# mschauer/ZigZagBoomerang.jl

Measured on AMD Instinct MI355X. Metric: reflection events/sec, d=16384 local ZigZag (spdmp), ensemble of independent chains, higher is better.
Workload: dtype f64

## Files before the change

include/pdmp_debug.h:

```cpp
#ifndef PDMP_DEBUG_H
#define PDMP_DEBUG_H

#include <stddef.h>

#include "pdmp_mi355.h"

#ifdef __cplusplus
extern "C" {
#endif

#define PDMP_DEBUG_KERNEL_AUTO 0
#define PDMP_DEBUG_KERNEL_SEQ 1
#define PDMP_DEBUG_KERNEL_SPEC4 2
#define PDMP_DEBUG_KERNEL_SPEC8 3
#define PDMP_DEBUG_KERNEL_EXACTP 4
pdmp_status pdmp_debug_set_kernel(pdmp_ensemble* ens, int kernel);
pdmp_status pdmp_debug_set_spec_g2(pdmp_ensemble* ens, int on);
pdmp_status pdmp_debug_set_phase_profile(pdmp_ensemble* ens, int on);
pdmp_status pdmp_debug_phase_profile(pdmp_ensemble* ens, double* out16, int* kind);
pdmp_status pdmp_debug_set_track_groups(pdmp_ensemble* ens, int which);
pdmp_status pdmp_debug_set_helper_wave(pdmp_ensemble* ens, int mode);
pdmp_status pdmp_debug_set_track_lines(pdmp_ensemble* ens, int mode);
pdmp_status pdmp_debug_buffer_addresses(pdmp_ensemble* ens, uint64_t* out8);
pdmp_status pdmp_debug_placement(pdmp_ensemble* ens, char* buf, size_t nbuf);
pdmp_status pdmp_debug_set_placement(pdmp_ensemble* ens, int tune, int place, const char* rec, const char* kp, const char* ev);
pdmp_status pdmp_debug_move_buffer(pdmp_ensemble* ens, int which);
pdmp_status pdmp_debug_set_helper_steering(pdmp_ensemble* ens, double gain, int target, double ahead);
pdmp_status pdmp_debug_set_launch_count_limit(pdmp_ensemble* ens, uint32_t n);
pdmp_status pdmp_debug_set_consumer_overlap(pdmp_ensemble* ens, int mode);
pdmp_status pdmp_debug_host_drain_probe(pdmp_ensemble* ens, int64_t bytes, double* gbps);
pdmp_status pdmp_debug_last_kernel(pdmp_ensemble* ens, char* out, int64_t cap);
pdmp_status pdmp_debug_set_logistic_rows(pdmp_ensemble* ens, int row_width);
pdmp_status pdmp_debug_set_proposal_dump(pdmp_ensemble* ens, int64_t n);

pdmp_status pdmp_debug_math_probe(int device, uint64_t seed, int64_t n, double* out);

#define PDMP_MATH_U01 0
#define PDMP_MATH_LOG 1
#define PDMP_MATH_EXP 2
#define PDMP_MATH_SINCOS 3
#define PDMP_MATH_SINCOS2PI 4
#define PDMP_MATH_RANDN 5
#define PDMP_MATH_RANDN2 6
#define PDMP_MATH_RANDINT 7
#define PDMP_MATH_DIV 8
#define PDMP_MATH_SQRT 9
#define PDMP_MATH_PT_DEV 16
#define PDMP_MATH_PT_DEV_L 17
#define PDMP_MATH_PT_BPS 18
#define PDMP_MATH_PT_BPS_L 19
#define PDMP_MATH_PT_D1 20
#define PDMP_MATH_PT_G 21
#define PDMP_MATH_PT_G_L 22
#define PDMP_MATH_PT_Q 23
// ... 40 lines not shown
```

zigzagboomerang.jl_amd/_lib.py:

```python
import ctypes as C
import os

import numpy as np

from . import build as _build

PDMP_OK = 0
ABI_VERSION = 3
ERR_NAMES = {0: "PDMP_OK", 1: "PDMP_ERR_INVALID", 2: "PDMP_ERR_NO_DEVICE", 3: "PDMP_ERR_HIP",
             4: "PDMP_ERR_UNSUPPORTED", 5: "PDMP_ERR_NOMEM"}

PDMP_ERR_INVALID, PDMP_ERR_NO_DEVICE, PDMP_ERR_HIP, PDMP_ERR_UNSUPPORTED, PDMP_ERR_NOMEM = 1, 2, 3, 4, 5
SAMPLER_ZIGZAG_LOCAL, SAMPLER_ZIGZAG_ALL, SAMPLER_BPS, SAMPLER_STICKY_ZIGZAG, SAMPLER_BARRIER_ZIGZAG = 0, 1, 2, 3, 4
BARRIER_RULES = {"sticky": 0, "reflect": 1, "reversible": 2}
BARRIER_FN_PT3_L, BARRIER_FN_HIT, BARRIER_FN_RATES = 0, 1, 2
CHAIN_OK, CHAIN_BOUND_VIOLATED, CHAIN_STALLED, CHAIN_TRACE_FULL, CHAIN_PAUSED = 0, 1, 2, 3, 4


def needs_rerun(status):
    st = np.asarray(status)
    return bool(np.any((st == CHAIN_TRACE_FULL) | (st == CHAIN_PAUSED)))
RUN_REFERENCE_TAIL, RUN_STOP_BEFORE = 0, 1

EVENT_DTYPE = np.dtype([("t", "<f8"), ("i", "<i8"), ("x", "<f8"), ("theta", "<f8")])
COUNTERS_DTYPE = np.dtype([("t_last", "<f8"), ("num", "<u8"), ("nacc", "<u8"), ("nrefresh", "<u8"),
                           ("ntrace", "<u8"), ("nevents", "<u8"), ("ndraw_main", "<u8"),
                           ("ndraw_global", "<u8"), ("status", "<u4"), ("reserved", "<u4")])
assert EVENT_DTYPE.itemsize == 32 and COUNTERS_DTYPE.itemsize == 72

EXPORTED_SYMBOLS = [
    "pdmp_last_error", "pdmp_abi_version", "pdmp_device_count", "pdmp_ensemble_create",
    "pdmp_ensemble_destroy", "pdmp_ensemble_set_flow_zigzag", "pdmp_ensemble_set_target_gaussian_csc",
    "pdmp_ensemble_set_state", "pdmp_ensemble_set_state_synthetic", "pdmp_ensemble_run", "pdmp_ensemble_run_partitioned", "pdmp_ensemble_sync",
    "pdmp_ensemble_last_run_ms", "pdmp_ensemble_counters", "pdmp_ensemble_totals", "pdmp_ensemble_trace_copy",
    "pdmp_ensemble_trace_reset", "pdmp_ensemble_final_state", "pdmp_ensemble_batch_means",
    "pdmp_ensemble_trace_dev", "pdmp_ensemble_counters_dev", 
    "pdmp_ensemble_set_flow_bps", "pdmp_ensemble_set_state_bps", "pdmp_ensemble_bps_trace_copy",
    "pdmp_ensemble_bps_final_state", "pdmp_ensemble_set_sticky", "pdmp_ensemble_set_adaptscale", "pdmp_ensemble_final_sigma", "pdmp_ensemble_set_flow_boomerang", "pdmp_ensemble_set_local_bound", "pdmp_ensemble_set_target_logistic", "pdmp_ensemble_set_flow_factboomerang",
    "pdmp_ensemble_set_mass_cholesky", "pdmp_ensemble_set_bps_options", "pdmp_ensemble_set_bps_moments", "pdmp_ensemble_bps_moments",
    "pdmp_ensemble_set_bps_sticky", "pdmp_ensemble_bps_trace_free_copy", "pdmp_ensemble_bps_final_sticky",
    "pdmp_ensemble_set_flow_bps_modern", "pdmp_ensemble_set_bps_record_limit", "pdmp_ensemble_set_target_bps_logistic",
    "pdmp_ensemble_set_barriers", "pdmp_ensemble_final_barrier", "pdmp_ensemble_set_target_diffusion_bridge",
    "pdmp_ensemble_ess_begin", "pdmp_ensemble_ess_batch", "pdmp_ensemble_ess_end", "pdmp_ensemble_set_gradient_tracking",
    "pdmp_ensemble_path_integrals", "pdmp_ensemble_set_path_integrals", "pdmp_ensemble_set_neighbourhood", "pdmp_ensemble_info",
    "pdmp_ensemble_consume_begin", "pdmp_ensemble_consume", "pdmp_ensemble_consume_async", "pdmp_ensemble_last_consume_ms", "pdmp_ensemble_consume_mean", "pdmp_ensemble_consume_inclusion", "pdmp_ensemble_consume_discretized", "pdmp_ensemble_consume_cummean", "pdmp_ensemble_consume_cummean_copy", "pdmp_ensemble_subtrace_copy", "pdmp_1d_run",
    "pdmp_ensemble_bps_consume_begin", "pdmp_ensemble_bps_consume", "pdmp_ensemble_bps_consume_mean", "pdmp_ensemble_bps_consume_inclusion",
    "pdmp_ensemble_bps_consume_discretized", "pdmp_ensemble_bps_consume_cummean", "pdmp_ensemble_bps_consume_cummean_copy",
    "pdmp_ensemble_consume_condition", "pdmp_ensemble_consume_conditioned", "pdmp_ensemble_bps_consume_condition", "pdmp_ensemble_bps_consume_conditioned",
    "pdmp_ensemble_consume_pairs", "pdmp_ensemble_consume_pair_integrals", "pdmp_ensemble_bps_consume_pairs", "pdmp_ensemble_bps_consume_pair_integrals",
    "pdmp_comm_unique_id", "pdmp_comm_init", "pdmp_comm_destroy", "pdmp_comm_info", "pdmp_comm_barrier", "pdmp_comm_allreduce",
    "pdmp_ensemble_gather_traces", "pdmp_ensemble_reduce_moments", "pdmp_comm_gathered_copy",
    "pdmp_ensemble_gather_bps_traces", "pdmp_comm_gathered_bps_copy", "pdmp_ensemble_bps_trace_dev",
]
DEBUG_SYMBOLS = ["pdmp_debug_set_kernel", "pdmp_debug_set_spec_g2", "pdmp_debug_set_phase_profile", "pdmp_debug_phase_profile",
                 "pdmp_debug_set_proposal_dump", "pdmp_debug_set_track_groups", "pdmp_debug_set_helper_wave", "pdmp_debug_set_track_lines", "pdmp_debug_buffer_addresses", "pdmp_debug_placement", "pdmp_debug_set_placement", "pdmp_debug_move_buffer", "pdmp_debug_set_helper_steering", "pdmp_debug_set_launch_count_limit", "pdmp_debug_host_drain_probe", "pdmp_debug_set_consumer_overlap", "pdmp_debug_last_kernel", "pdmp_debug_set_logistic_rows", "pdmp_debug_math_probe", "pdmp_debug_math_eval", "pdmp_debug_write_probe", "pdmp_debug_sector_probe",
                 "pdmp_debug_sticky_eval", "pdmp_debug_trace_append", "pdmp_debug_barrier_eval", "pdmp_debug_bps_trace_append"]
DEBUG_KERNELS = {"auto": 0, "seq": 1, "spec4": 2, "spec8": 3, "exactp": 4}


class PdmpConfig(C.Structure):
    _fields_ = [("struct_size", C.c_uint32), ("device", C.c_int32), ("sampler", C.c_int32), ("adapt", C.c_int32),
                ("factor", C.c_double), ("nchains", C.c_int64), ("d", C.c_int64), ("trace_capacity", C.c_int64)]


class PdmpError(RuntimeError):
    def __init__(self, code, msg):
        super().__init__(f"{ERR_NAMES.get(code, code)}: {msg}")
        self.code = code


_lib = None
_loaded_path = None


def loaded_path():
    return _loaded_path


def lib_path():
    return os.environ.get("PDMP_MI355_LIB") or _build.LIB_PATH


def load():
    global _lib, _loaded_path
    if _lib is not None:
        return _lib
    path = lib_path()
    if not os.path.exists(path):
# ... 86 lines not shown
    L.pdmp_ensemble_set_local_bound.argtypes = [vp, C.c_int]
    L.pdmp_ensemble_set_gradient_tracking.argtypes = [vp, C.c_int]
    L.pdmp_ensemble_final_sigma.argtypes = [vp, i64, i64, vp]
    L.pdmp_ensemble_set_flow_bps.argtypes = [vp, vp, vp, vp, vp, f64, f64]
    L.pdmp_ensemble_set_flow_boomerang.argtypes = [vp, vp, vp, vp, vp, vp, f64, f64]
    L.pdmp_ensemble_set_state_bps.argtypes = [vp, f64, vp, vp, f64, vp]
    L.pdmp_ensemble_ess_begin.argtypes = [vp, f64]
    L.pdmp_ensemble_ess_batch.argtypes = [vp, f64]
    L.pdmp_ensemble_ess_end.argtypes = [vp, vp, vp, vp, vp, C.POINTER(i64), C.POINTER(f64), C.POINTER(f64)]
    L.pdmp_ensemble_set_mass_cholesky.argtypes = [vp, vp, vp, vp]
    L.pdmp_ensemble_set_bps_options.argtypes = [vp, C.c_int, C.c_int]
    L.pdmp_ensemble_set_bps_moments.argtypes = [vp, C.c_int]
    L.pdmp_ensemble_bps_moments.argtypes = [vp, f64, i64, i64, vp, vp]
    L.pdmp_ensemble_set_bps_sticky.argtypes = [vp, vp, C.c_int]
    L.pdmp_ensemble_bps_trace_free_copy.argtypes = [vp, i64, i64, i64, vp]
    L.pdmp_ensemble_bps_final_sticky.argtypes = [vp, i64, i64, vp, vp]
    L.pdmp_ensemble_set_flow_bps_modern.argtypes = [vp, C.c_double, C.c_double, vp, C.c_int]
    L.pdmp_ensemble_set_target_bps_logistic.argtypes = [vp, i64, vp, vp, vp, vp, vp, vp, vp, vp, f64]
    L.pdmp_ensemble_set_bps_record_limit.argtypes = [vp, i64]
    L.pdmp_debug_sticky_eval.argtypes = [C.c_int, C.c_int, i64, vp, vp, vp, vp]
    L.pdmp_debug_barrier_eval.argtypes = [C.c_int, C.c_int, i64, vp, vp, vp, vp]
    L.pdmp_ensemble_set_barriers.argtypes = [vp, vp, vp, vp, vp, vp, vp, C.c_int]
    L.pdmp_ensemble_final_barrier.argtypes = [vp, i64, i64, vp, vp]
    L.pdmp_debug_trace_append.argtypes = [vp, i64, vp, i64]
    L.pdmp_ensemble_bps_trace_copy.argtypes = [vp, i64, i64, i64, vp, vp, vp]
    L.pdmp_ensemble_bps_final_state.argtypes = [vp, i64, i64, vp, vp, vp, vp]
    L.pdmp_debug_set_kernel.argtypes = [vp, C.c_int]
    L.pdmp_debug_set_spec_g2.argtypes = [vp, C.c_int]
    L.pdmp_debug_set_phase_profile.argtypes = [vp, C.c_int]
    L.pdmp_debug_phase_profile.argtypes = [vp, vp, C.POINTER(C.c_int)]
    L.pdmp_debug_set_proposal_dump.argtypes = [vp, i64]
    L.pdmp_debug_set_track_groups.argtypes = [vp, C.c_int]
    L.pdmp_debug_set_helper_wave.argtypes = [vp, C.c_int]
    L.pdmp_debug_set_track_lines.argtypes = [vp, C.c_int]
    L.pdmp_debug_buffer_addresses.argtypes = [vp, C.POINTER(C.c_uint64)]
    L.pdmp_debug_move_buffer.argtypes = [vp, C.c_int]
    L.pdmp_debug_placement.argtypes = [vp, C.c_char_p, C.c_size_t]
    L.pdmp_debug_set_placement.argtypes = [vp, C.c_int, C.c_int, C.c_char_p, C.c_char_p, C.c_char_p]
    L.pdmp_debug_set_launch_count_limit.argtypes = [vp, C.c_uint32]
    L.pdmp_debug_set_helper_steering.argtypes = [vp, C.c_double, C.c_int, C.c_double]
    L.pdmp_debug_last_kernel.argtypes = [vp, C.c_char_p, i64]
    L.pdmp_debug_set_logistic_rows.argtypes = [vp, C.c_int]
    for name in EXPORTED_SYMBOLS + DEBUG_SYMBOLS:
        fn = getattr(L, name)
        if name not in ("pdmp_last_error", "pdmp_abi_version", "pdmp_device_count", "pdmp_ensemble_destroy", "pdmp_comm_destroy"):
            fn.restype = C.c_int
    _lib = L
    _loaded_path = path
    return L


class Config1d(C.Structure):
    _fields_ = [("struct_size", C.c_uint32), ("device", C.c_int32), ("flow", C.c_int32), ("adapt", C.c_int32), ("factor", C.c_double),
                ("nchains", C.c_int64), ("trace_capacity", C.c_int64), ("mu", C.c_double), ("sigma2", C.c_double), ("noise", C.c_double),
                ("b_sigma", C.c_double), ("b_mu", C.c_double), ("b_lambda", C.c_double)]


EVENT1D_DTYPE = np.dtype([("t", "<f8"), ("x", "<f8"), ("theta", "<f8")])
STATE1D_DTYPE = np.dtype([("t", "<f8"), ("x", "<f8"), ("theta", "<f8"), ("c", "<f8"), ("a", "<f8"), ("b", "<f8"), ("t_next", "<f8"),
                          ("t_ref", "<f8"), ("ndraw", "<u8"), ("num", "<i8"), ("acc", "<i8"), ("started", "<i4"), ("status", "<i4")])


def check(code):
    if code != PDMP_OK:
        raise PdmpError(code, load().pdmp_last_error().decode("utf-8", "replace"))

# ... 40 lines not shown
```

zigzagboomerang.jl_amd/csrc/pdmp_capi.hip:

```cpp
#include <algorithm>
#include <cstdarg>
#include <cstdio>
#include <cstring>

#include "pdmp_ensemble.hpp"

namespace {
thread_local std::string g_err;
thread_local std::string g_deferred_err;
}

pdmp_status fail(pdmp_status st, const char* fmt, ...) {
    char buf[512];
    va_list ap;
    va_start(ap, fmt);
    vsnprintf(buf, sizeof buf, fmt, ap);
    va_end(ap);
    g_err = buf;
    return st;
}
pdmp_status fail_hip(const char* expr, hipError_t err) {
    const std::string dm = g_deferred_err;
    g_deferred_err.clear();
    return fail(PDMP_ERR_HIP, "%s failed: %s%s%s", expr, hipGetErrorString(err), dm.empty() ? "" : " -- ", dm.c_str());
// ... 261 lines not shown
        return fail(PDMP_ERR_UNSUPPORTED, "PDMP_DEBUG_KERNEL_EXACTP: spdmp on a plain lattice (16 <= n <= 128, d >= 2048) with the bounding matrix equal to the target's, no adaptation, and a trace or no trace");
#endif
    const bool sticky_spec = sticky && e->use_spec && e->blob_mmax <= 16 && !dump;
    *fam = sticky ? (sticky_spec ? FAM_STICKY_SPEC : FAM_STICKY_RUN) : spec_ok ? FAM_SPEC : FAM_ONE_EVENT;
    return PDMP_OK;
}

pdmp_status ensemble_run_impl(pdmp_ensemble* e, double T, int flags, void* stream) {
    if (!e) return fail(PDMP_ERR_INVALID, "null argument");
    if (!e->has_state) return fail(PDMP_ERR_INVALID, "set_state must be called before run");
    if (e->trace_appended) return fail(PDMP_ERR_INVALID, "pdmp_debug_trace_append was used on this ensemble: its records no longer match its trace (set_state first)");
    if (flags != PDMP_RUN_REFERENCE_TAIL && flags != PDMP_RUN_STOP_BEFORE) return fail(PDMP_ERR_INVALID, "bad flags");
    HIP_TRY(hipSetDevice(e->cfg.device));
    e->ran = true;
    hipStream_t s = stream ? (hipStream_t)stream : e->stream;
    const int64_t n = e->cfg.nchains;
    const bool bps = e->cfg.sampler == PDMP_SAMPLER_BPS;
    if (!bps) e->dbg_phase_valid = 0;
    if (!bps && general_path(e) && e->lg_nemax >= 1024 && !e->d_hot.p) PDMP_TRY(e->d_hot.alloc((size_t)n * (size_t)e->cfg.d * 4));
    const pdmp::BpsRunParams B = bps_run_params(e, T, flags);
    pdmp::ZzRunParams P = run_params(e, T, flags);
    const pdmp::ZzGeneralParams Q = general_params(e);
    const pdmp::ZzLogisticTables LT = logistic_tables(e);
    KernelFamily fam;
    PDMP_TRY(select_family(e, P, Q, LT, &fam));
    const FamilyInfo& F = FAMILY[fam];
    DevBuf<double> dbgbuf, phbuf;
    const int64_t dbg_cap = bps ? 0 : e->dbg_dump;
    if (dbg_cap > 0) {
        PDMP_TRY(dbgbuf.alloc((size_t)dbg_cap * 16));
        HIP_TRY(hipMemsetAsync(dbgbuf.p, 0, (size_t)dbg_cap * 16 * sizeof(double), s));
        P.dbg = dbgbuf.p;
        P.dbg_cap = dbg_cap;
    }
    HIP_TRY(hipEventRecord(e->ev0, s));
    const bool profiled = e->dbg_phase != 0 && F.phase_kind != 0;
    if (profiled) {
        PDMP_TRY(phbuf.alloc(16));
        HIP_TRY(hipMemsetAsync(phbuf.p, 0, 16 * sizeof(double), s));
        P.dbg = phbuf.p;
        P.dbg_cap = 0;
    }
    int rc = 0;
    switch (fam) {
    case FAM_BPS:
        if (e->bps.modern && e->bps.logit) {
            e->last_kernel = "bps_logit_run_kernel";
            rc = pdmp::launch_bps_logit_run(B, bps_modern_params(e), bps_logit_params(e), n, s);
        } else if (e->bps.modern) {
            e->last_kernel = "bps_modern_run_kernel";
            rc = pdmp::launch_bps_modern_run(B, bps_modern_params(e), n, s);
        } else if (e->bps.sticky) {
            e->last_kernel = "bps_sticky_run_kernel";
            rc = pdmp::launch_bps_sticky_run(B, bps_sticky_params(e), n, s);
        } else {
            e->last_kernel = "bps_run_kernel";
            rc = pdmp::launch_bps_run(B, n, e->bps.diag, s, bps_moments_params(e));
        }
        break;
    case FAM_GENERAL: e->last_kernel = "zz_general_run_kernel"; rc = pdmp::launch_zz_general_run(P, Q, n, s); break;
    case FAM_LOGISTIC_LDS: e->last_kernel = "zz_logistic_lds_kernel"; rc = pdmp::launch_zz_logistic_lds(P, Q, LT, e->keep_integrals, n, s); break;
    case FAM_TRACKL: e->last_kernel = "zz_local_trackl_kernel"; e->canon_stale = true; rc = pdmp::launch_zz_local_trackl(P, n, s); break;
    case FAM_TRACKP: rc = pdmp::launch_zz_local_trackp(P, n, s, &e->last_kernel); break;
    case FAM_TRACK_GROUPS: e->last_kernel = "zz_local_track_kernel"; rc = pdmp::launch_zz_local_track(P, n, s); break;
    case FAM_STICKY_SPEC: e->last_kernel = "zz_sticky_spec_kernel"; rc = pdmp::launch_zz_sticky_spec(P, n, s); break;
    case FAM_STICKY_RUN: e->last_kernel = "zz_sticky_run_kernel"; rc = pdmp::launch_zz_sticky_run(P, n, s); break;
// ... 354 lines not shown
```

zigzagboomerang.jl_amd/csrc/pdmp_capi_debug.hip:

```cpp
#include <algorithm>
#include <chrono>
#include <cstdio>
#include <cstring>

#include "pdmp_ensemble.hpp"

template <class Launch>
static pdmp_status time_launches(const char* name, int iters, double* ms_out, Launch launch) {
    hipEvent_t e0, e1;
    HIP_TRY(hipEventCreate(&e0));
    HIP_TRY(hipEventCreate(&e1));
    (void)launch();
    HIP_TRY(hipEventRecord(e0, nullptr));
    for (int k = 0; k < iters; ++k) LAUNCH_TRY_CODE(name, launch());
    HIP_TRY(hipEventRecord(e1, nullptr));
    HIP_TRY(hipEventSynchronize(e1));
    float ms = 0.f;
    HIP_TRY(hipEventElapsedTime(&ms, e0, e1));
    *ms_out = (double)ms / iters;
    (void)hipEventDestroy(e0);
    (void)hipEventDestroy(e1);
    return PDMP_OK;
}

// ... 170 lines not shown
    if (!e || !e->has_state) return fail(PDMP_ERR_INVALID, "move buffer: an ensemble with a state");
    if ((which >= 6) != (e->cfg.sampler == PDMP_SAMPLER_BPS)) return fail(PDMP_ERR_INVALID, "move buffer: 6-10 are the Bouncy Particle's arrays, 0-5 the ZigZag's");
    HIP_TRY(device_sync(e));
    auto move_buf = [](auto& b) -> hipError_t {
        if (!b.p || b.n == 0) return hipSuccess;
        void* np = nullptr;
        const size_t bytes = b.n * sizeof(*b.p);
        hipError_t r = hipMalloc(&np, bytes);
        if (r != hipSuccess) return r;
        r = hipMemcpy(np, b.p, bytes, hipMemcpyDeviceToDevice);
        if (r != hipSuccess) return r;
        b.p = static_cast<decltype(b.p)>(np);
        return hipSuccess;
    };
    switch (which) {
        case 0: HIP_TRY(move_buf(e->d_rec)); break;
        case 1: HIP_TRY(move_buf(e->d_kp)); break;
        case 2: HIP_TRY(move_buf(e->d_ev)); break;
        case 3: HIP_TRY(move_buf(e->d_hdr)); break;
        case 4: HIP_TRY(move_buf(e->d_cc)); break;
        case 5: HIP_TRY(move_buf(e->d_keys)); break;
        case 6: HIP_TRY(move_buf(e->b_ev_x)); break;
        case 7: HIP_TRY(move_buf(e->b_ev_th)); break;
        case 8: HIP_TRY(move_buf(e->b_x)); break;
        case 9: HIP_TRY(move_buf(e->b_th)); break;
        case 10: HIP_TRY(move_buf(e->b_ev_t)); break;
        default: return fail(PDMP_ERR_INVALID, "move buffer: 0 records, 1 pairs, 2 trace, 3 headers, 4 constants, 5 keys; BPS: 6 / 7 event x / theta, 8 / 9 x / theta, 10 event t");
    }
    return PDMP_OK;
}
pdmp_status pdmp_debug_set_helper_wave(pdmp_ensemble* e, int mode) {
    if (!e || mode < -1 || mode > 1) return fail(PDMP_ERR_INVALID, "helper wave: -1 (by occupancy), 0 (never), 1 (always)");
    e->dbg_helper_wave = mode;
    return PDMP_OK;
}
pdmp_status pdmp_debug_set_consumer_overlap(pdmp_ensemble* e, int mode) {
    if (!e || mode < -1 || mode > 1) return fail(PDMP_ERR_INVALID, "consumer overlap: -1 (by width), 0 (between slices), 1 (beside the next slice)");
    e->dbg_cons_overlap = mode;
    return PDMP_OK;
}
pdmp_status pdmp_debug_set_launch_count_limit(pdmp_ensemble* e, uint32_t n) {
    if (!e) return fail(PDMP_ERR_INVALID, "null argument");
    e->dbg_count_limit = n;
    return PDMP_OK;
}
pdmp_status pdmp_debug_set_helper_steering(pdmp_ensemble* e, double gain, int target, double ahead) {
    if (!e || !(gain > 0.0 && gain <= 4096.0) || target < 1 || target > 64 || !(ahead >= 0.0))
        return fail(PDMP_ERR_INVALID, "helper steering: 0 < gain <= 4096 (<= 1 for the two-wave form), 1 <= target <= 64, ahead >= 0");
    e->dbg_hw_steer[0] = gain;
    e->dbg_hw_steer[1] = (double)target;
    e->dbg_hw_steer[2] = ahead;
    return PDMP_OK;
}
pdmp_status pdmp_debug_set_logistic_rows(pdmp_ensemble* e, int w) {
    if (!e || (w != -1 && w != 0 && w != 16 && w != 32)) return fail(PDMP_ERR_INVALID, "row width: -1 (default), 0 (one chain per wavefront), 16 or 32");
#ifndef PDMP_EXTRA_KERNELS
    if (w > 0) return fail(PDMP_ERR_UNSUPPORTED, "zz_logistic_rows_kernel is not part of this library: it lives in the parity build (build.py --variant parity, -DPDMP_EXTRA_KERNELS)");
#endif
    e->dbg_lg_rows = w;
    return PDMP_OK;
}
pdmp_status pdmp_debug_set_proposal_dump(pdmp_ensemble* e, int64_t n) {
    if (!e || n < 0) return fail(PDMP_ERR_INVALID, "bad argument");
    e->dbg_dump = n;
    return PDMP_OK;
}
// ... 111 lines not shown
```

zigzagboomerang.jl_amd/csrc/pdmp_engine.hpp:

```cpp
#pragma once
#include <cstdint>
#include <string>
#include <vector>

#include "../../include/pdmp_mi355.h"
#ifdef PDMP_EXTRA_KERNELS
#include "../../include/pdmp_debug.h"
#endif

namespace pdmp {

struct alignas(64) ZzRec {
    double x;
    double th;
    double t;
    double I;
    double t_old;
    double a, b;
    uint64_t acc;
};
static_assert(sizeof(ZzRec) == 64, "record must be one 64-byte sector");

struct alignas(128) TrRec {
    double x, th, tx, I;
// ... 41 lines not shown
    h.c.t_last = t0;
    h.c.num = 0;
    h.c.nacc = 0;
    h.c.nrefresh = 0;
    h.c.ntrace = ntrace;
    h.c.nevents = nevents;
    h.c.ndraw_main = ndraw_main;
    h.c.ndraw_global = 0;
    h.c.status = PDMP_CHAIN_OK;
    h.c.reserved = 0;
    h.seed = seed;
    h.t0 = t0;
    h.t_event = t0;
    h.tl_scale = 0.0;
    for (int k = 0; k < 3; ++k) h.pad[k] = 0;
    return h;
}

constexpr uint32_t PDMP_PRIO_TURN = 256u;
struct PrioTurn {
    uint32_t slot, it;
    __device__ __forceinline__ PrioTurn() : slot((uint32_t)__builtin_amdgcn_s_getreg(4 | (0 << 6) | (3 << 11)) & 3u), it(0) {}
    __device__ __forceinline__ void step() {
        if ((it & (PDMP_PRIO_TURN - 1u)) == 0u) {
            const uint32_t pr = ((it / PDMP_PRIO_TURN) + slot) & 3u;
            switch (pr) {
                case 0: __builtin_amdgcn_s_setprio(0); break;
                case 1: __builtin_amdgcn_s_setprio(1); break;
                case 2: __builtin_amdgcn_s_setprio(2); break;
                default: __builtin_amdgcn_s_setprio(3); break;
            }
        }
        it += 1;
    }
};
#endif

struct CoordConst {
    double c, c100;
    uint32_t cp, k;
    double gam[5];
};
static_assert(sizeof(CoordConst) == 64, "half a line");

struct BarrierEntry {
    double lo, hi;
    double klo, khi;
    uint32_t rules;
    uint32_t pad;
};
static_assert(sizeof(BarrierEntry) == 40, "barrier table entry");
constexpr uint64_t BARRIER_ACT_HIT = 0, BARRIER_ACT_REFLECT = 1, BARRIER_ACT_UNFREEZE = 2;

struct ZzTables {
    const uint32_t* __restrict__ colptr;
    const uint32_t* __restrict__ rowval;
    const double* __restrict__ bval;
    const double* __restrict__ tval;
    const double* __restrict__ gmu_b;
    const double* __restrict__ gmu_t;
    const uint32_t* __restrict__ sptr;
    const uint32_t* __restrict__ sidx;
    const uint32_t* __restrict__ qptr;
    const uint8_t* __restrict__ pos;
    const uint8_t* __restrict__ selfpos;
    const double* __restrict__ c_shared;
// ... 10 lines not shown
    ZzTables tb;
    ZzRec* rec;
    double* keys;
    DevChain* hdr;
    pdmp_event* ev;
    double* c_chain;
    double* dbg;
    int64_t dbg_cap;
    const uint64_t* __restrict__ blob;
    const uint32_t* __restrict__ tix;
    uint32_t blob_w, blob_w_pad, blob_sw, blob_pw, blob_kmax;
    uint32_t common_tix;
    int64_t d;
    int64_t dk;
    int64_t trace_cap;
    uint32_t nblk;
    uint32_t nblk_pad;
    double T;
    double factor;
    double lambda_ref;
    int32_t flags;
    int32_t adapt;
    int32_t has_refresh;
    int32_t move_all;
    int32_t force_spec4;
    int32_t track_two_sums;
    int32_t track_mean;
    uint32_t count_limit;
    uint32_t typ_extra;
    double hw_gain, hw_ahead;
    uint32_t hw_target;
    int32_t n_cu;
    int32_t helper_wave;
    void* tl_lines;
    void* tl_cold;
    int32_t lattice_n;
    uint32_t lattice_magic;
    const uint64_t* __restrict__ g8_line;
    const double* __restrict__ g8_member;
    const double* __restrict__ g8_gamt;
    int32_t g8_gw;
    const double* __restrict__ kappa;
    double* thf;
    int32_t reversible, strong_upperbounds;
    const BarrierEntry* __restrict__ barriers;
};

struct ZzInitParams {
    ZzTables tb;
    ZzRec* rec;
    double* keys;
    DevChain* hdr;
    double* c_chain;
    const double* x0;
    const double* th0;
    const uint64_t* seeds;
    uint64_t seed0;
    int64_t d;
    int64_t dk;
    int64_t nchains;
    double t0;
    double lambda_ref;
    int32_t has_refresh;
    int32_t sticky;
    double* thf;
    int32_t flow_kind;
// ... 340 lines not shown
```

zigzagboomerang.jl_amd/csrc/pdmp_ensemble.hpp:

```cpp
#pragma once
#include <hip/hip_runtime.h>

#include <cstdint>
#include <string>
#include <vector>

#include "../../include/pdmp_debug.h"
#include "pdmp_engine.hpp"

#pragma GCC visibility push(hidden)

pdmp_status fail(pdmp_status st, const char* fmt, ...);
pdmp_status fail_hip(const char* expr, hipError_t err);
pdmp_status fail_launch(const char* launcher, int rc, bool hip_rc);

#define HIP_TRY(expr)                                    \
    do {                                                 \
        hipError_t e_ = (expr);                          \
        if (e_ != hipSuccess) return fail_hip(#expr, e_); \
    } while (0)
#define LAUNCH_TRY_AS(name, rc, hip_rc)                            \
    do {                                                           \
        const int rc_ = (rc);                                      \
        if (rc_ != 0) return fail_launch(name, rc_, hip_rc);       \
// ... 176 lines not shown
    DevBuf<unsigned char> d_pr_cur, d_pr_meta;
    bool pr_on = false;
    int64_t pr_np = 0;
    bool trace_appended = false;
    DevBuf<pdmp_event> d_ev2;
    DevBuf<uint64_t> d_snap[2];
    hipStream_t stream2 = nullptr;
    hipEvent_t ev_run_done = nullptr, ev_cons_done[2] = {nullptr, nullptr}, ev_c0 = nullptr, ev_c1 = nullptr;
    bool cons_pending[2] = {false, false}, cons_timed = false;
    int async_k = 0;
    pdmp_event* deferred_buf = nullptr;
    int deferred_k = -1;

    DevBuf<double> d_jprev, d_sum, d_jstart, d_essacc;
    double ess_T0 = 0.0, ess_Tlast = 0.0;
    int64_t ess_batches = -1;

    pdmp::PlaceConfig place_cfg;
    int place_tune = 1;
    std::string tune_log;

    int dbg_kernel = 0;
    int dbg_lg_rows = -1;
    int dbg_spec_g2 = 0;
    int dbg_phase = 0;
    double dbg_phase_out[16] = {0};
    int dbg_phase_valid = 0;
    int64_t dbg_dump = 0;
    int dbg_track_groups = 0;
    double dbg_hw_steer[3] = {0, 0, 0};
    uint32_t dbg_count_limit = 0;
    int dbg_cons_overlap = -1;
    int dbg_helper_wave = -1;
    int dbg_track_lines = -1;

    BpsOptions bps;
    DevBuf<int64_t> b_colptr, b_rowval, bt_colptr, bt_rowval;
    DevBuf<double> b_nzval, b_mu, b_mu_flow, b_x, b_th, b_scal, b_ev_t, b_ev_x, b_ev_th, bt_nzval, bt_mu;
    DevBuf<int32_t> m_Lcp, m_Lrv, m_Ucp, m_Urv;
    DevBuf<double> m_Lnz, m_Unz;
    DevBuf<double> b_j1, b_j2;
    DevBuf<double> b_jT, b_jT2;
    DevBuf<double> b_kappa, b_thf, b_tfrez;
    DevBuf<uint64_t> b_fmask, b_ev_f;
    DevBuf<double> b_udiag, b_sudiag, b_mstate;
    DevBuf<int64_t> bl_Acp, bl_Arv, bl_Atcp, bl_Atrv;
    DevBuf<double> bl_Anz, bl_Atnz, bl_y, bl_m, bl_eta;
    int64_t bl_n = 0;
    double bl_gamma0 = 0.0;
    DevBuf<double> bc_cur, bc_grid, bc_cm;
    DevBuf<unsigned char> bc_meta;
    bool bc_on = false, bc_cummean = false;
    double bc_dt = 0.0;
    int64_t bc_K = 0;
    DevBuf<double> bcn_pn, bcn_tau, bcn_t, bcn_x;
    DevBuf<unsigned long long> bcn_nh;
    bool bcn_on = false, bc_started = false;
    int64_t bcn_max_hits = 0;

    DevBuf<int32_t> bpr_pi, bpr_pj;
    DevBuf<double> bpr_c, bpr_S, bpr_J, bpr_T;
    bool bpr_on = false;
    int64_t bpr_np = 0;

    pdmp::ZzTables tables() const {
        pdmp::ZzTables tb{};
// ... 64 lines not shown
```

zigzagboomerang.jl_amd/csrc/pdmp_trackp.hip:

```cpp
#include <hip/hip_runtime.h>

#include <cstdint>

#include "../../include/pdmp_detmath.h"
#include "pdmp_device.hpp"
#include "pdmp_engine.hpp"

namespace pdmp {

namespace {

__device__ __forceinline__ uint32_t w_grp8_min_u32(uint32_t v) {
    uint32_t o = (uint32_t)__builtin_amdgcn_mov_dpp((int)v, 0xB1, 0xf, 0xf, true);
    v = (o < v) ? o : v;
    o = (uint32_t)__builtin_amdgcn_mov_dpp((int)v, 0x4E, 0xf, 0xf, true);
    v = (o < v) ? o : v;
    o = (uint32_t)__builtin_amdgcn_mov_dpp((int)v, 0x141, 0xf, 0xf, true);
    return (o < v) ? o : v;
}
__device__ __forceinline__ uint32_t p_enc(double key, double tb, uint32_t pos) {
    double dlt = key - tb;
    dlt = (dlt > 0.0) ? dlt : 0.0;
    const uint32_t b = __float_as_uint((float)dlt);
    return (((b >= 8u) ? b - 8u : 0u) & ~7u) | pos;
// ... 11 lines not shown
    return reinterpret_cast<const uint32_t*>(smem)[b] & 7u;
}

}

template <bool HW, bool BIG = false>
struct WL {
    static_assert(!(HW && BIG), "the two-wave form keeps 2048 block bounds");
    static constexpr uint32_t NBLK = BIG ? 8192 : 2048;
    static constexpr uint32_t XO = (NBLK - 2048) * 4;
    static constexpr uint32_t LB = 0;
    static constexpr uint32_t EX = XO + 8192;
    static constexpr uint32_t URING = XO + 8704;
    static constexpr uint32_t SLB = XO + (HW ? 9792 : 9728);
    static constexpr uint32_t TB = XO + (HW ? 9920 : 9856);
    static constexpr uint32_t ACL = XO + (HW ? 10048 : 9984);
    static constexpr uint32_t NB = XO + (HW ? 10144 : 10016);
    static constexpr uint32_t CTL = 10272;
    static constexpr uint32_t HPF = 10336;
    static constexpr uint32_t RING = 10464;
    static constexpr int CMAX = HW ? 64 : 56;
    static constexpr uint32_t WIN = HW ? 256u : 128u;
    static constexpr uint32_t BYTES = HW ? RING + 512 * 16 : NB + 128;
};
constexpr uint32_t W_NR = 512;
constexpr uint32_t W_BYTES_1W = WL<false>::BYTES, W_BYTES_BIG = WL<false, true>::BYTES;
constexpr uint32_t W_BYTES_HW = WL<true>::BYTES;
constexpr int W_AMAX = 8;
#ifndef W_GROW
#define W_GROW 1.02
#define W_SHRINK 0.98
#define W_SLACK 5u
#endif
#define W_TARGET_HW 48u
#define W_GAIN_HW 0.3
#define W_TARGET_1W 44u
#define W_TARGET_1W_MAX_PER_CU 12
#define W_NHYP 8
#define W_NHYP_1W 4
#define W_PF_AHEAD 1.0
static_assert(WL<false>::BYTES <= 10240, "16 chains per CU: 160 KB / 16");
static_assert(WL<false>::URING + WL<false>::WIN * 8 <= WL<false>::SLB && WL<false, true>::URING + WL<false, true>::WIN * 8 <= WL<false, true>::SLB &&
                  WL<false>::ACL + W_AMAX * 2 <= WL<false>::NB,
              "the one-wave forms' ring of draws ends where the event blocks begin");
static_assert(WL<false, true>::BYTES <= 40960, "d <= 65536: 4 chains per CU (one per SIMD), 160 KB / 4");
static_assert(W_BYTES_HW == WL<true>::RING + W_NR * 16 && W_BYTES_HW <= 20480, "8 chains per CU: 160 KB / 8");
struct WCtl {
    uint32_t filled;
    uint32_t consumed;
    uint32_t exitf;
    uint32_t pad;
    double pf_tau, pf_dt, pf_tb;
};
typedef volatile __attribute__((address_space(3))) WCtl* WCtlPtr;
__device__ __forceinline__ WCtlPtr w_ctl(unsigned char* smem, uint32_t offset) {
    return (WCtlPtr)(__attribute__((address_space(3))) unsigned char*)(smem + offset);
}

namespace {
__device__ __forceinline__ bool nb_has(const uint4 nb, uint32_t v2) {
    const uint32_t x0 = nb.x ^ v2, x1 = nb.y ^ v2, x2 = nb.z ^ v2, x3 = nb.w ^ v2;
    const uint32_t z = ((x0 - 0x00010001u) & ~x0) | ((x1 - 0x00010001u) & ~x1) | ((x2 - 0x00010001u) & ~x2) | ((x3 - 0x00010001u) & ~x3);
    return (z & 0x80008000u) != 0u;
}
__device__ __forceinline__ uint32_t nb_count(const uint4 nb) {
    const uint64_t hi = ((uint64_t)nb.w << 32) | nb.z, lo = ((uint64_t)nb.y << 32) | nb.x;
// ... 107 lines not shown
    if (status == PDMP_CHAIN_BOUND_VIOLATED || status == PDMP_CHAIN_STALLED) return;
    const uint64_t seed = hdr->seed;
    const uint64_t nm0 = hdr->c.ndraw_main, ntrace0 = hdr->c.ntrace;
    if (HW) {
        if (threadIdx.x == 0) {
            ctl->filled = 0u;
            ctl->consumed = 0u;
            ctl->exitf = 0u;
            ctl->pf_tau = -PDMP_INF;
            ctl->pf_dt = 0.0;
            ctl->pf_tb = 0.0;
        }
        __syncthreads();
        if (threadIdx.x >= 64) {
            trackp_helper<LAT>(P, smem, lane, chain, seed, nm0);
            return;
        }
    }
    uint32_t dnm = 0, dnum = 0, dnacc = 0, vnacc = 0;
    double unext = 0.0;
    uint32_t ufilled = 0, uflushed = 0;
    bool uhave = false;
    double t_last = hdr->c.t_last;
    double t_event = hdr->t_event;
    status = PDMP_CHAIN_OK;
    const double T = P.T;
    const bool stop_before = (P.flags & PDMP_RUN_STOP_BEFORE) != 0;
    const uint32_t trace_room = (P.trace_cap > 0)
                                    ? (uint32_t)(((uint64_t)P.trace_cap > ntrace0) ? ((uint64_t)P.trace_cap - ntrace0) : 0)
                                    : 0xffffffffu;

    double seldt = 1e-3;
    double tb;
    {
        double mloc = t_last;
        for (uint32_t b = lane; b < nblk; b += 64) {
            const double2* p = kp + (size_t)b * 8;
#pragma unroll
            for (int q = 0; q < 8; ++q) mloc = min_f64(mloc, p[q].x);
        }
        tb = wave_min_f64(mloc);
    }
    for (uint32_t b = lane; b < W_NBLK; b += 64) {
        uint32_t e = P_INFBITS;
        if (b < nblk) {
            const double2* p = kp + (size_t)b * 8;
            double mk = p[0].x;
            uint32_t mi = 0;
#pragma unroll
            for (int q = 1; q < 8; ++q) {
                const double v = p[q].x;
                if (v < mk) {
                    mk = v;
                    mi = q;
                }
            }
            e = (mk < PDMP_INF) ? p_enc(mk, tb, mi) : P_INFBITS;
        }
        lbf[b] = e;
    }
    PDMP_LDS_ORDER();

    uint64_t ph[10] = {0, 0, 0, 0, 0, 0, 0, 0, 0, 0};
    uint64_t ph_t0 = PROF ? (uint64_t)__builtin_readcyclecounter() : 0;
    uint64_t ph_rounds = 0, ph_guess = 0;
    uint64_t ph_iters = 0, ph_raw = 0, ph_zone = 0, ph_eval = 0;
#ifdef PDMP_PHASE_MARKS
#define WMARK(k) asm volatile("; WPHASE " #k)
#else
#define WMARK(k)
#endif
#define WPHASE(k)                                                         \
    do {                                                                  \
        WMARK(k);                                                         \
        if (PROF) {                                                       \
            const uint64_t now_ = (uint64_t)__builtin_readcyclecounter(); \
            ph[k] += now_ - ph_t0;                                        \
            ph_t0 = now_;                                                 \
        }                                                                 \
    } while (0)

    PrioTurn prio;
    bool need_rebase = false;
    uint32_t idle = 0;
    bool running = stop_before || (t_event < T);
    while (running) {
        prio.step();
        if (dnacc >= trace_room) {
            status = PDMP_CHAIN_TRACE_FULL;
            break;
        }
        if (dnm >= P.count_limit) {
            status = PDMP_CHAIN_PAUSED;
            break;
        }
        if (HW) {
            if (lane == 0) ctl->consumed = dnm;
            while (ctl->filled < dnm + W_WIN) __builtin_amdgcn_s_sleep(1);
            PDMP_LDS_ORDER();
        } else {
            const uint32_t ulim = dnm + W_WIN;
            while (ufilled < ulim) {
                const uint32_t n = ufilled + (uint32_t)lane;
                if (!uhave) {
                    unext = pdmp_u01(seed, PDMP_STREAM_MAIN, nm0 + (uint64_t)n);
                    uhave = true;
                }
                const uint32_t uend = (ufilled + 64u < ulim) ? ufilled + 64u : ulim;
                if (n >= uflushed && n < uend) uring[n & (W_WIN - 1u)] = unext;
                uflushed = uend;
                if (uend != ufilled + 64u) break;
                ufilled += 64u;
                uhave = false;
            }
            PDMP_LDS_ORDER();
        }
        WPHASE(7);
        auto draw = [&](uint32_t n) -> double {
            if (HW) return ring[n & (W_NR - 1u)].x;
            return uring[n & (W_WIN - 1u)];
// ... 692 lines not shown
            const uint32_t costL = (uint32_t)__builtin_amdgcn_readlane((int)cost, (int)(Rc - 1u));
            const uint32_t offL = (uint32_t)__builtin_amdgcn_readlane((int)off, (int)(Rc - 1u));
            dnum += Rc;
            idle = 0;
            dnacc += (uint32_t)__popcll(acc_c);
            dnm += offL + costL;
            t_last = readlane_f64(tp, (int)(Rc - 1u));
            if (acc_c) t_event = readlane_f64(tp, 63 - __builtin_clzll(acc_c));
        }
        if (vsel >= 0) {
            const double tpv = readlane_f64(tp, vsel);
            const uint32_t iv = (uint32_t)__builtin_amdgcn_readlane((int)i, vsel);
            if (lane == 0) kp[iv].y = tpv;
            dnum += 1;
            vnacc = 1;
            dnm += 1;
            t_last = tpv;
            status = PDMP_CHAIN_BOUND_VIOLATED;
        }
        if (status != PDMP_CHAIN_OK) break;
        PDMP_LDS_ORDER();
    }

    if (PROF && P.dbg && chain == 0 && lane == 0) {
        for (int q = 0; q < 10; ++q) P.dbg[q] = (double)ph[q];
        P.dbg[10] = (double)ph_iters;
        P.dbg[11] = (double)ph_raw;
        P.dbg[12] = (double)ph_zone;
        P.dbg[13] = (double)ph_eval;
        P.dbg[14] = (double)ph_rounds;
        P.dbg[15] = (double)ph_guess;
    }
#undef WPHASE
    if (HW && lane == 0) ctl->exitf = 1u;
    if (lane == 0) {
        hdr->c.t_last = t_last;
        hdr->t_event = t_event;
        hdr->c.num += dnum;
        hdr->c.nacc += dnacc + vnacc;
        hdr->c.ntrace = ntrace0 + dnacc;
        hdr->c.nevents += dnacc;
        hdr->c.ndraw_main = nm0 + dnm;
        hdr->c.status = status;
    }
}

template <bool PROF, bool LAT>
__global__ __launch_bounds__(64) __attribute__((amdgpu_waves_per_eu(4, 4))) void zz_local_trackp_kernel(ZzRunParams P) {
    trackp_body<PROF, LAT, false, false>(P);
}
template <bool PROF>
__global__ __launch_bounds__(64) __attribute__((amdgpu_waves_per_eu(1, 2))) void zz_local_trackp_big_kernel(ZzRunParams P) {
    trackp_body<PROF, true, false, true>(P);
}
template <bool PROF, bool LAT>
__global__ __launch_bounds__(128) __attribute__((amdgpu_waves_per_eu(4, 4))) void zz_local_trackp2_kernel(ZzRunParams P) {
    trackp_body<PROF, LAT, true, false>(P);
}

bool zz_trackp_supported(const ZzRunParams& p) {
    const bool lattice = p.lattice_n >= 16 && p.lattice_n <= 256 && p.d <= (int64_t)WL<false, true>::NBLK * 8;
    const bool graph = p.lattice_n == 0 && p.tb.nb16 != nullptr && p.tb.gam8 != nullptr && p.d <= (int64_t)WL<false>::NBLK * 8;
    return (lattice || graph) && p.tb.gmu_t == nullptr && !p.track_two_sums && !p.has_refresh && p.d >= 2048;
}

bool zz_trackp_big(int64_t d) { return d > (int64_t)WL<false>::NBLK * 8; }
// ... 114 lines not shown
```

zigzagboomerang.jl_amd/engine.py:

```python
import ctypes as C
import os

import numpy as np

from . import _lib
from .flows import BouncyParticle, DiffusionBridgeTarget, FactBoomerang, GaussianTarget, LogisticRegressionTarget, LogisticTarget, ZigZag


def _i64(a):
    return np.ascontiguousarray(a, dtype=np.int64)


def _f64(a):
    return np.ascontiguousarray(a, dtype=np.float64)


def _ptr(a):
    return None if a is None else a.ctypes.data


class Ensemble:

    def __init__(self, nchains, d, *, sampler=_lib.SAMPLER_ZIGZAG_LOCAL, adapt=False, factor=1.8, device=0,
                 trace_capacity=0):
        self._L = _lib.load()
        self.nchains, self.d = int(nchains), int(d)
        self.trace_capacity = int(trace_capacity)
        self.adapt = bool(adapt)
        self.device = int(device)
        self._bps_mom = 0
        cfg = _lib.PdmpConfig(C.sizeof(_lib.PdmpConfig), int(device), int(sampler), int(bool(adapt)), float(factor),
                              self.nchains, self.d, self.trace_capacity)
        h = C.c_void_p()
        _lib.check(self._L.pdmp_ensemble_create(C.byref(cfg), C.byref(h)))
        self._h = h
        k = os.environ.get("PDMP_KERNEL")
        if k:
            self.debug_set_kernel(k)
        if os.environ.get("PDMP_TRACK_GROUPS"):
            _lib.check(self._L.pdmp_debug_set_track_groups(self._h, int(os.environ["PDMP_TRACK_GROUPS"])))
        if os.environ.get("PDMP_HELPER_WAVE"):
            self.debug_set_helper_wave(int(os.environ["PDMP_HELPER_WAVE"]))
        if os.environ.get("PDMP_TRACK_LINES"):
            self.debug_set_track_lines(int(os.environ["PDMP_TRACK_LINES"]))
        if any(os.environ.get(v) for v in ("PDMP_PLACE_TUNE", "PDMP_PLACE", "PDMP_PLACE_rec", "PDMP_PLACE_kp", "PDMP_PLACE_ev")):
            pat = [os.environ.get("PDMP_PLACE_" + a, "").encode() or None for a in ("rec", "kp", "ev")]
            self.debug_set_placement(int(os.environ.get("PDMP_PLACE_TUNE", "-1")), int(os.environ.get("PDMP_PLACE", "1" if any(pat) else "0")), *pat)
        if os.environ.get("PDMP_LAUNCH_COUNT_LIMIT"):
            _lib.check(self._L.pdmp_debug_set_launch_count_limit(self._h, int(os.environ["PDMP_LAUNCH_COUNT_LIMIT"])))
        if os.environ.get("PDMP_HELPER_STEER"):
            g_, k_, a_ = os.environ["PDMP_HELPER_STEER"].split(",")
            _lib.check(self._L.pdmp_debug_set_helper_steering(self._h, float(g_), int(k_), float(a_)))
        if os.environ.get("PDMP_LG_ROWS"):
            _lib.check(self._L.pdmp_debug_set_logistic_rows(self._h, int(os.environ["PDMP_LG_ROWS"])))
        if os.environ.get("PDMP_SPEC_G2"):
            _lib.check(self._L.pdmp_debug_set_spec_g2(self._h, 1))

    def debug_set_kernel(self, name):
        _lib.check(self._L.pdmp_debug_set_kernel(self._h, _lib.DEBUG_KERNELS[name]))

    def debug_set_helper_wave(self, mode):
        _lib.check(self._L.pdmp_debug_set_helper_wave(self._h, int(mode)))

    def debug_set_track_lines(self, mode):
        _lib.check(self._L.pdmp_debug_set_track_lines(self._h, int(mode)))

    def debug_buffer_addresses(self):
        import ctypes as C
        out = (C.c_uint64 * 8)()
        _lib.check(self._L.pdmp_debug_buffer_addresses(self._h, out))
        return dict(zip(("trk", "kp", "ev", "hdr", "rec", "keys", "cc", "blob"), [int(v) for v in out]))

    def debug_set_placement(self, tune=-1, place=0, rec=None, kp=None, ev=None):
        _lib.check(self._L.pdmp_debug_set_placement(self._h, int(tune), int(place), rec, kp, ev))

    def debug_placement(self):
        import ctypes
        buf = ctypes.create_string_buffer(1024)
        _lib.check(self._L.pdmp_debug_placement(self._h, buf, 1024))
        return buf.value.decode()

    def debug_move_buffer(self, which):
        _lib.check(self._L.pdmp_debug_move_buffer(self._h, int(which)))

    def kernel_name(self):
        import ctypes
        buf = ctypes.create_string_buffer(96)
        _lib.check(self._L.pdmp_debug_last_kernel(self._h, buf, 96))
        return buf.value.decode()

    def debug_set_logistic_rows(self, row_width):
        _lib.check(self._L.pdmp_debug_set_logistic_rows(self._h, int(row_width)))

    def debug_phase_profile(self, on=True):
        _lib.check(self._L.pdmp_debug_set_phase_profile(self._h, int(bool(on))))
# ... 510 lines not shown
```

Measured before the change: 1.401 billion.

## Set wave priority by progress rank among co-resident chains; one-pass block-min init

Replaces the round-robin wave priority rotation in the track-P kernel with a progress-aware policy. Each wave periodically publishes its normalized simulated time to a device board row keyed by XCC/CU/SIMD, reads its neighbours' entries and sets s_setprio so the most-lagging chains get the highest priority, which aims to cut tail imbalance across the ensemble. It also rewrites the initial per-block minimum/argmin pass as a single unrolled, software-pipelined sweep using group-of-8 shuffles, instead of two separate loops over kp. This adds periodic atomics and a board allocation, and relies on hardware register IDs to choose the board row, so it risks slot collisions and extra overhead.

```diff
diff --git a/include/pdmp_debug.h b/include/pdmp_debug.h
--- a/include/pdmp_debug.h
+++ b/include/pdmp_debug.h
@@ -20,6 +20,7 @@
 pdmp_status pdmp_debug_phase_profile(pdmp_ensemble* ens, double* out16, int* kind);
 pdmp_status pdmp_debug_set_track_groups(pdmp_ensemble* ens, int which);
 pdmp_status pdmp_debug_set_helper_wave(pdmp_ensemble* ens, int mode);
+pdmp_status pdmp_debug_set_prio_policy(pdmp_ensemble* ens, int mode);
 pdmp_status pdmp_debug_set_track_lines(pdmp_ensemble* ens, int mode);
 pdmp_status pdmp_debug_buffer_addresses(pdmp_ensemble* ens, uint64_t* out8);
 pdmp_status pdmp_debug_placement(pdmp_ensemble* ens, char* buf, size_t nbuf);
diff --git a/zigzagboomerang.jl_amd/_lib.py b/zigzagboomerang.jl_amd/_lib.py
--- a/zigzagboomerang.jl_amd/_lib.py
+++ b/zigzagboomerang.jl_amd/_lib.py
@@ -53,7 +53,7 @@
     "pdmp_ensemble_gather_bps_traces", "pdmp_comm_gathered_bps_copy", "pdmp_ensemble_bps_trace_dev",
 ]
 DEBUG_SYMBOLS = ["pdmp_debug_set_kernel", "pdmp_debug_set_spec_g2", "pdmp_debug_set_phase_profile", "pdmp_debug_phase_profile",
-                 "pdmp_debug_set_proposal_dump", "pdmp_debug_set_track_groups", "pdmp_debug_set_helper_wave", "pdmp_debug_set_track_lines", "pdmp_debug_buffer_addresses", "pdmp_debug_placement", "pdmp_debug_set_placement", "pdmp_debug_move_buffer", "pdmp_debug_set_helper_steering", "pdmp_debug_set_launch_count_limit", "pdmp_debug_host_drain_probe", "pdmp_debug_set_consumer_overlap", "pdmp_debug_last_kernel", "pdmp_debug_set_logistic_rows", "pdmp_debug_math_probe", "pdmp_debug_math_eval", "pdmp_debug_write_probe", "pdmp_debug_sector_probe",
+                 "pdmp_debug_set_proposal_dump", "pdmp_debug_set_track_groups", "pdmp_debug_set_helper_wave", "pdmp_debug_set_prio_policy", "pdmp_debug_set_track_lines", "pdmp_debug_buffer_addresses", "pdmp_debug_placement", "pdmp_debug_set_placement", "pdmp_debug_move_buffer", "pdmp_debug_set_helper_steering", "pdmp_debug_set_launch_count_limit", "pdmp_debug_host_drain_probe", "pdmp_debug_set_consumer_overlap", "pdmp_debug_last_kernel", "pdmp_debug_set_logistic_rows", "pdmp_debug_math_probe", "pdmp_debug_math_eval", "pdmp_debug_write_probe", "pdmp_debug_sector_probe",
                  "pdmp_debug_sticky_eval", "pdmp_debug_trace_append", "pdmp_debug_barrier_eval", "pdmp_debug_bps_trace_append"]
 DEBUG_KERNELS = {"auto": 0, "seq": 1, "spec4": 2, "spec8": 3, "exactp": 4}
 
@@ -206,6 +206,7 @@
     L.pdmp_debug_set_proposal_dump.argtypes = [vp, i64]
     L.pdmp_debug_set_track_groups.argtypes = [vp, C.c_int]
     L.pdmp_debug_set_helper_wave.argtypes = [vp, C.c_int]
+    L.pdmp_debug_set_prio_policy.argtypes = [vp, C.c_int]
     L.pdmp_debug_set_track_lines.argtypes = [vp, C.c_int]
     L.pdmp_debug_buffer_addresses.argtypes = [vp, C.POINTER(C.c_uint64)]
     L.pdmp_debug_move_buffer.argtypes = [vp, C.c_int]
diff --git a/zigzagboomerang.jl_amd/csrc/pdmp_capi.hip b/zigzagboomerang.jl_amd/csrc/pdmp_capi.hip
--- a/zigzagboomerang.jl_amd/csrc/pdmp_capi.hip
+++ b/zigzagboomerang.jl_amd/csrc/pdmp_capi.hip
@@ -317,6 +317,15 @@
         HIP_TRY(hipMemsetAsync(dbgbuf.p, 0, (size_t)dbg_cap * 16 * sizeof(double), s));
         P.dbg = dbgbuf.p;
         P.dbg_cap = dbg_cap;
+    }
+    if (fam == FAM_TRACKP && e->dbg_prio_policy != 0) {
+        if (!e->d_prio_board.p) {
+            PDMP_TRY(e->d_prio_board.alloc(pdmp::PDMP_PRIO_BOARD_WORDS));
+            HIP_TRY(hipMemsetAsync(e->d_prio_board.p, 0, (size_t)pdmp::PDMP_PRIO_BOARD_WORDS * sizeof(uint32_t), s));
+        }
+        e->prio_epoch = e->prio_epoch % 255u + 1u;
+        P.prio_board = e->d_prio_board.p;
+        P.prio_epoch = e->prio_epoch;
     }
     HIP_TRY(hipEventRecord(e->ev0, s));
     const bool profiled = e->dbg_phase != 0 && F.phase_kind != 0;
diff --git a/zigzagboomerang.jl_amd/csrc/pdmp_capi_debug.hip b/zigzagboomerang.jl_amd/csrc/pdmp_capi_debug.hip
--- a/zigzagboomerang.jl_amd/csrc/pdmp_capi_debug.hip
+++ b/zigzagboomerang.jl_amd/csrc/pdmp_capi_debug.hip
@@ -226,6 +226,11 @@
 pdmp_status pdmp_debug_set_helper_wave(pdmp_ensemble* e, int mode) {
     if (!e || mode < -1 || mode > 1) return fail(PDMP_ERR_INVALID, "helper wave: -1 (by occupancy), 0 (never), 1 (always)");
     e->dbg_helper_wave = mode;
+    return PDMP_OK;
+}
+pdmp_status pdmp_debug_set_prio_policy(pdmp_ensemble* e, int mode) {
+    if (!e || mode < -1 || mode > 1) return fail(PDMP_ERR_INVALID, "priority policy: -1 (default: by rank of progress where it applies), 0 (in turns), 1 (by rank of progress)");
+    e->dbg_prio_policy = mode;
     return PDMP_OK;
 }
 pdmp_status pdmp_debug_set_consumer_overlap(pdmp_ensemble* e, int mode) {
diff --git a/zigzagboomerang.jl_amd/csrc/pdmp_engine.hpp b/zigzagboomerang.jl_amd/csrc/pdmp_engine.hpp
--- a/zigzagboomerang.jl_amd/csrc/pdmp_engine.hpp
+++ b/zigzagboomerang.jl_amd/csrc/pdmp_engine.hpp
@@ -97,6 +97,54 @@
             }
         }
         it += 1;
+    }
+};
+
+#ifndef PDMP_PRIO_LAG_K
+#define PDMP_PRIO_LAG_K 32u
+#endif
+constexpr uint32_t PDMP_PRIO_BOARD_ROWS = 1u << 15, PDMP_PRIO_BOARD_SLOTS = 16u;
+constexpr uint32_t PDMP_PRIO_BOARD_WORDS = PDMP_PRIO_BOARD_ROWS * PDMP_PRIO_BOARD_SLOTS;
+struct PrioLag {
+    PrioTurn turn;
+    uint32_t* row;
+    uint32_t slot, tag, it;
+    double t_begin, scale;
+    __device__ __forceinline__ PrioLag(uint32_t* board, uint32_t epoch, double t_begin_, double T) : row(nullptr), slot(0), tag(epoch << 24), it(0), t_begin(t_begin_), scale(0.0) {
+        const double span = T - t_begin_;
+        if (board != nullptr && epoch != 0u && span > 0.0 && span < __builtin_inf()) {
+            const uint32_t xcc = (uint32_t)__builtin_amdgcn_s_getreg(20 | (0 << 6) | (3 << 11));
+            const uint32_t hw = (uint32_t)__builtin_amdgcn_s_getreg(4 | (4 << 6) | (11 << 11));
+            slot = (uint32_t)__builtin_amdgcn_s_getreg(4 | (0 << 6) | (3 << 11)) & (PDMP_PRIO_BOARD_SLOTS - 1u);
+            row = board + (size_t)(((xcc << 12) | hw) & (PDMP_PRIO_BOARD_ROWS - 1u)) * PDMP_PRIO_BOARD_SLOTS;
+            scale = 16777216.0 / span;
+        }
+    }
+    __device__ __forceinline__ void step(double t_last, int lane) {
+        if (row == nullptr) {
+            turn.step();
+            return;
+        }
+        if ((it & (PDMP_PRIO_LAG_K - 1u)) == 0u) {
+            const double f = (t_last - t_begin) * scale;
+            const uint32_t q = (f > 0.0) ? ((f < 16777214.0) ? (uint32_t)f : 0xfffffeu) : 0u;
+            if (lane == 0) __hip_atomic_store(row + slot, tag | q, __ATOMIC_RELAXED, __HIP_MEMORY_SCOPE_AGENT);
+            uint32_t w = 0u;
+            if (lane < (int)PDMP_PRIO_BOARD_SLOTS) w = __hip_atomic_load(row + lane, __ATOMIC_RELAXED, __HIP_MEMORY_SCOPE_AGENT);
+            const uint32_t wq = w & 0xffffffu;
+            const bool behind = lane < (int)PDMP_PRIO_BOARD_SLOTS && (w & 0xff000000u) == tag && wq != 0xffffffu && (wq < q || (wq == q && (uint32_t)lane < slot));
+            const uint32_t rank = (uint32_t)__popcll(__ballot(behind));
+            switch (rank) {
+                case 0: __builtin_amdgcn_s_setprio(3); break;
+                case 1: __builtin_amdgcn_s_setprio(2); break;
+                case 2: __builtin_amdgcn_s_setprio(1); break;
+                default: __builtin_amdgcn_s_setprio(0); break;
+            }
+        }
+        it += 1;
+    }
+    __device__ __forceinline__ void finish(int lane) {
+        if (row != nullptr && lane == 0) __hip_atomic_store(row + slot, tag | 0xffffffu, __ATOMIC_RELAXED, __HIP_MEMORY_SCOPE_AGENT);
     }
 };
 #endif
@@ -173,6 +221,8 @@
     uint32_t hw_target;
     int32_t n_cu;
     int32_t helper_wave;
+    uint32_t* prio_board;
+    uint32_t prio_epoch;
     void* tl_lines;
     void* tl_cold;
     int32_t lattice_n;
diff --git a/zigzagboomerang.jl_amd/csrc/pdmp_ensemble.hpp b/zigzagboomerang.jl_amd/csrc/pdmp_ensemble.hpp
--- a/zigzagboomerang.jl_amd/csrc/pdmp_ensemble.hpp
+++ b/zigzagboomerang.jl_amd/csrc/pdmp_ensemble.hpp
@@ -232,6 +232,9 @@
     uint32_t dbg_count_limit = 0;
     int dbg_cons_overlap = -1;
     int dbg_helper_wave = -1;
+    int dbg_prio_policy = -1;
+    DevBuf<uint32_t> d_prio_board;
+    uint32_t prio_epoch = 0;
     int dbg_track_lines = -1;
 
     BpsOptions bps;
diff --git a/zigzagboomerang.jl_amd/csrc/pdmp_trackp.hip b/zigzagboomerang.jl_amd/csrc/pdmp_trackp.hip
--- a/zigzagboomerang.jl_amd/csrc/pdmp_trackp.hip
+++ b/zigzagboomerang.jl_amd/csrc/pdmp_trackp.hip
@@ -67,6 +67,9 @@
 #define W_SHRINK 0.98
 #define W_SLACK 5u
 #endif
+#ifndef W_HEAD_ONE_PASS
+#define W_HEAD_ONE_PASS 1
+#endif
 #define W_TARGET_HW 48u
 #define W_GAIN_HW 0.3
 #define W_TARGET_1W 44u
@@ -240,7 +243,50 @@
 
     double seldt = 1e-3;
     double tb;
-    {
+    if (!BIG && W_HEAD_ONE_PASS) {
+        double bm[32];
+        uint32_t bpos[4] = {0u, 0u, 0u, 0u};
+        double mloc = t_last;
+        double vn[8];
+        auto load8 = [&](int s) {
+#pragma unroll
+            for (int j = 0; j < 8; ++j) {
+                const uint32_t k = 8u * (uint32_t)s + (uint32_t)j;
+                const bool in = 8u * k + (uint32_t)g < nblk;
+                const double v = kp[(in ? (size_t)64 * k : (size_t)0) + (size_t)lane].x;
+                vn[j] = in ? v : PDMP_INF;
+            }
+        };
+        load8(0);
+#pragma unroll
+        for (int s = 0; s < 32; ++s) {
+            double vc[8];
+#pragma unroll
+            for (int j = 0; j < 8; ++j) vc[j] = vn[j];
+            __builtin_amdgcn_sched_barrier(0);
+            if (s + 1 < 32) load8(s + 1);
+            __builtin_amdgcn_sched_barrier(0);
+            double keep = PDMP_INF;
+            uint32_t kpos = 0u;
+#pragma unroll
+            for (int j = 0; j < 8; ++j) {
+                const double v = vc[j];
+                const double m = grp8_min_f64(v);
+                const uint32_t pos = w_grp8_min_u32((v == m) ? (uint32_t)gl : 8u);
+                keep = (gl == j) ? m : keep;
+                kpos = (gl == j) ? pos : kpos;
+            }
+            asm volatile("" : "+v"(keep), "+v"(kpos));
+            bm[s] = keep;
+            bpos[s >> 3] |= (kpos & 7u) << (4 * (s & 7));
+            asm volatile("" : "+v"(bpos[s >> 3]));
+            mloc = min_f64(mloc, keep);
+        }
+        tb = wave_min_f64(mloc);
+#pragma unroll
+        for (int s = 0; s < 32; ++s)
+            lbf[64 * s + 8 * gl + g] = (bm[s] < PDMP_INF) ? p_enc(bm[s], tb, (bpos[s >> 3] >> (4 * (s & 7))) & 7u) : P_INFBITS;
+    } else {
         double mloc = t_last;
         for (uint32_t b = lane; b < nblk; b += 64) {
             const double2* p = kp + (size_t)b * 8;
@@ -248,24 +294,24 @@
             for (int q = 0; q < 8; ++q) mloc = min_f64(mloc, p[q].x);
         }
         tb = wave_min_f64(mloc);
-    }
-    for (uint32_t b = lane; b < W_NBLK; b += 64) {
-        uint32_t e = P_INFBITS;
-        if (b < nblk) {
-            const double2* p = kp + (size_t)b * 8;
-            double mk = p[0].x;
-            uint32_t mi = 0;
-#pragma unroll
-            for (int q = 1; q < 8; ++q) {
-                const double v = p[q].x;
-                if (v < mk) {
-                    mk = v;
-                    mi = q;
-                }
-            }
-            e = (mk < PDMP_INF) ? p_enc(mk, tb, mi) : P_INFBITS;
-        }
-        lbf[b] = e;
+        for (uint32_t b = lane; b < W_NBLK; b += 64) {
+            uint32_t e = P_INFBITS;
+            if (b < nblk) {
+                const double2* p = kp + (size_t)b * 8;
+                double mk = p[0].x;
+                uint32_t mi = 0;
+#pragma unroll
+                for (int q = 1; q < 8; ++q) {
+                    const double v = p[q].x;
+                    if (v < mk) {
+                        mk = v;
+                        mi = q;
+                    }
+                }
+                e = (mk < PDMP_INF) ? p_enc(mk, tb, mi) : P_INFBITS;
+            }
+            lbf[b] = e;
+        }
     }
     PDMP_LDS_ORDER();
 
@@ -288,12 +334,12 @@
         }                                                                 \
     } while (0)
 
-    PrioTurn prio;
+    PrioLag prio((!HW && !BIG) ? P.prio_board : nullptr, P.prio_epoch, t_last, T);
     bool need_rebase = false;
     uint32_t idle = 0;
     bool running = stop_before || (t_event < T);
     while (running) {
-        prio.step();
+        prio.step(t_last, lane);
         if (dnacc >= trace_room) {
             status = PDMP_CHAIN_TRACE_FULL;
             break;
@@ -1052,6 +1098,7 @@
         P.dbg[15] = (double)ph_guess;
     }
 #undef WPHASE
+    prio.finish(lane);
     if (HW && lane == 0) ctl->exitf = 1u;
     if (lane == 0) {
         hdr->c.t_last = t_last;
diff --git a/zigzagboomerang.jl_amd/engine.py b/zigzagboomerang.jl_amd/engine.py
--- a/zigzagboomerang.jl_amd/engine.py
+++ b/zigzagboomerang.jl_amd/engine.py
@@ -41,6 +41,8 @@
             _lib.check(self._L.pdmp_debug_set_track_groups(self._h, int(os.environ["PDMP_TRACK_GROUPS"])))
         if os.environ.get("PDMP_HELPER_WAVE"):
             self.debug_set_helper_wave(int(os.environ["PDMP_HELPER_WAVE"]))
+        if os.environ.get("PDMP_PRIO_POLICY"):
+            self.debug_set_prio_policy(int(os.environ["PDMP_PRIO_POLICY"]))
         if os.environ.get("PDMP_TRACK_LINES"):
             self.debug_set_track_lines(int(os.environ["PDMP_TRACK_LINES"]))
         if any(os.environ.get(v) for v in ("PDMP_PLACE_TUNE", "PDMP_PLACE", "PDMP_PLACE_rec", "PDMP_PLACE_kp", "PDMP_PLACE_ev")):
@@ -61,6 +63,9 @@
 
     def debug_set_helper_wave(self, mode):
         _lib.check(self._L.pdmp_debug_set_helper_wave(self._h, int(mode)))
+
+    def debug_set_prio_policy(self, mode):
+        _lib.check(self._L.pdmp_debug_set_prio_policy(self._h, int(mode)))
 
     def debug_set_track_lines(self, mode):
         _lib.check(self._L.pdmp_debug_set_track_lines(self._h, int(mode)))
```

After: 1.450 billion (median of 6 runs). +3.4%, better.
